# ReaganCardoza/Physics-Based-Ray-Tracing

Measured on AMD Instinct MI355X. Metric: Msamples/s on cbox.xml 512x512 x 256 spp (radiance, path max_depth 6), higher is better.
Workload: dtype f32

## Files before the change

include/pbrt_hip.h:

```cpp
#ifndef PBRT_HIP_H
#define PBRT_HIP_H

#include <stdint.h>

#ifdef __cplusplus
extern "C" {
#endif

#define PBRT_ABI_VERSION 5

#define PBRT_OK 0
#define PBRT_E_INVALID (-1)
#define PBRT_E_DEVICE (-2)
#define PBRT_E_NOMEM (-3)
#define PBRT_E_UNSUPPORTED (-4)

#define PBRT_PRIM_TRIANGLE 0u
#define PBRT_PRIM_SPHERE 1u
#define PBRT_PRIM_PARALLELOGRAM 2u
#define PBRT_PRIM_CONE 3u
#define PBRT_PRIM_CYLINDER 4u

typedef struct pbrt_prim {
    float g[12];
// ... 34 lines not shown
#define PBRT_ACCEL_BVH 2u
#define PBRT_ACCEL_BVH_GLOBAL 3u

typedef struct pbrt_scene_desc {
    uint32_t n_prims;
    const pbrt_prim *prims;
    uint32_t n_materials;
    const pbrt_material *materials;
    uint32_t n_emitters;
    const pbrt_emitter *emitters;
    uint32_t n_light_prims;
    const uint32_t *light_prims;
    const float *light_cdf;
    uint32_t accel;
    const float *vertex_normals;
} pbrt_scene_desc;

typedef struct pbrt_camera {
    float to_world[12];
    float tan_half_fov_x;
    float near_clip;
    float far_clip;
    uint32_t film_w;
    uint32_t film_h;
} pbrt_camera;

#define PBRT_FILTER_BOX 0u
#define PBRT_FILTER_TENT 1u
#define PBRT_FILTER_GAUSSIAN 2u

typedef struct pbrt_film_desc {
    uint32_t crop_x, crop_y, crop_w, crop_h;
    uint32_t spp;
    uint32_t sample_offset;
    uint32_t max_depth;
    uint32_t rr_depth;
    uint32_t filter;
    uint32_t seed;
    uint32_t flags;
    uint32_t pass_paths;
} pbrt_film_desc;

#define PBRT_FILM_RAW_ACCUM 1u
#define PBRT_FILM_NO_REPACK 2u
#define PBRT_FILM_FUSE_PLAN_SET 0x80u
#define PBRT_FILM_FUSE_PLAN(mask) (PBRT_FILM_FUSE_PLAN_SET | (((mask) & 0xffu) << 8))
#define PBRT_FILM_WALK_SET 0x10000u
#define PBRT_FILM_WALK_FROM(d) (PBRT_FILM_WALK_SET | (((d) & 0xffu) << 17))
#define PBRT_FILM_REGEN 8u
#define PBRT_FILM_NO_HIT_POOL 0x10u
#define PBRT_FILM_NO_OCCLUDER_PRUNING 4u
#define PBRT_FILM_NO_TILE_CULL 0x20u
#define PBRT_FILM_NO_ORDERED_WALK 0x40u

#define PBRT_US_MAX_ANGLES 64

typedef struct pbrt_us_emitter {
    uint32_t number_of_elements;
    float pitch, element_width, element_height;
    float radius;
    float opening_angle;
    uint32_t number_of_rays_per_element;
    float speed_of_sound;
    float steering_angle_min, steering_angle_max;
} pbrt_us_emitter;

#define PBRT_US_PRIMARY_ELEMENT 0u
#define PBRT_US_PRIMARY_EMITTER 1u
#define PBRT_US_ARRAY_CONVEX 0x100u

typedef struct pbrt_us_params {
    uint32_t max_depth;
    float frequency;
    float sound_speed;
    float attenuation;
    float main_beam_angle;
    float cutoff_angle;
    float fs;
    uint32_t n_elements;
    float pitch;
    uint32_t n_angles;
    float angles_deg[PBRT_US_MAX_ANGLES];
    uint32_t time_samples;
    float sensor_to_world[12];
    float max_path_len;
    uint32_t quirks;
    uint32_t primary;
    pbrt_us_emitter emitter;
} pbrt_us_params;

#define PBRT_USQ_DIAG_SAMPLE 0x1u
#define PBRT_USQ_REF_REFLECT 0x2u
#define PBRT_USQ_UNIT_GGX_PDF 0x4u
#define PBRT_USQ_DOUBLE_LOCAL 0x8u
#define PBRT_USQ_MIXED_FRAMES 0x10u
#define PBRT_USQ_NEVER_ENTER 0x20u
#define PBRT_USQ_CLAMP_TIME 0x40u
#define PBRT_USQ_NO_TOF_ACCUM 0x80u
#define PBRT_USQ_NO_CARRIER 0x100u
#define PBRT_USQ_NO_FIRST_TABLES 0x200u
#define PBRT_USQ_NO_FUSED_BOUNCES 0x400u
#define PBRT_USQ_FROZEN_DRAWS 0x800u
#define PBRT_USQ_SIGNED_RR 0x1000u
#define PBRT_USQ_DRJIT_VARIANT (PBRT_USQ_CLAMP_TIME | PBRT_USQ_NO_TOF_ACCUM | PBRT_USQ_FROZEN_DRAWS | PBRT_USQ_SIGNED_RR)
#define PBRT_USQ_REFERENCE                                                                \
    (PBRT_USQ_DIAG_SAMPLE | PBRT_USQ_REF_REFLECT | PBRT_USQ_UNIT_GGX_PDF | PBRT_USQ_DOUBLE_LOCAL | \
// ... 266 lines not shown
```

physics-based-ray-tracing_amd/_capi.py:

```python
from __future__ import annotations

import contextlib
import ctypes as C
import os
import sys

import numpy as np

_HERE = os.path.dirname(os.path.abspath(__file__))
LIB_PATH = os.environ.get("PBRT_HIP_LIB") or os.path.join(_HERE, "csrc", "libpbrt_hip.so")

PBRT_ABI_VERSION = 5

PRIM_TRIANGLE, PRIM_SPHERE, PRIM_PARALLELOGRAM, PRIM_CONE, PRIM_CYLINDER = 0, 1, 2, 3, 4
MAT_DIFFUSE, MAT_CONDUCTOR, MAT_DIELECTRIC, MAT_ULTRA, MAT_NONE = 0, 1, 2, 3, 4
MAT_ROUGHCONDUCTOR, MAT_CONDUCTOR_FRESNEL = 5, 6
EMIT_AREA, EMIT_POINT = 0, 1
ACCEL_AUTO, ACCEL_BRUTE, ACCEL_BVH, ACCEL_BVH_GLOBAL = 0, 1, 2, 3
FILTER_BOX, FILTER_TENT, FILTER_GAUSSIAN = 0, 1, 2
FILM_RAW_ACCUM = 1
FILM_NO_REPACK = 2
FILM_NO_OCCLUDER_PRUNING = 4
FILM_NO_TILE_CULL = 0x20
FILM_NO_ORDERED_WALK = 0x40
FILM_NO_HIT_POOL = 0x10
FILM_REGEN = 8
FILM_FUSE_PLAN_SET = 0x80


FILM_WALK_SET = 0x10000


def film_walk_from(depth: int) -> int:
    return FILM_WALK_SET | ((int(depth) & 0xFF) << 17)


def film_fuse_plan(mask: int) -> int:
    return FILM_FUSE_PLAN_SET | ((int(mask) & 0xFF) << 8)

US_MAX_ANGLES = 64

USQ_DIAG_SAMPLE = 0x1
USQ_REF_REFLECT = 0x2
USQ_UNIT_GGX_PDF = 0x4
USQ_DOUBLE_LOCAL = 0x8
USQ_MIXED_FRAMES = 0x10
USQ_NEVER_ENTER = 0x20
USQ_CLAMP_TIME = 0x40
USQ_NO_TOF_ACCUM = 0x80
USQ_NO_CARRIER = 0x100
USQ_NO_FIRST_TABLES = 0x200
USQ_NO_FUSED_BOUNCES = 0x400
USQ_FROZEN_DRAWS = 0x800
USQ_SIGNED_RR = 0x1000
USQ_DRJIT_VARIANT = USQ_CLAMP_TIME | USQ_NO_TOF_ACCUM | USQ_FROZEN_DRAWS | USQ_SIGNED_RR
USQ_REFERENCE = (USQ_DIAG_SAMPLE | USQ_REF_REFLECT | USQ_UNIT_GGX_PDF | USQ_DOUBLE_LOCAL
                 | USQ_MIXED_FRAMES | USQ_NEVER_ENTER)

PRIM_DTYPE = np.dtype([("g", np.float32, 12), ("type", np.uint32), ("material", np.uint32),
                       ("emitter", np.int32), ("shape", np.uint32)])
MATERIAL_DTYPE = np.dtype([("type", np.uint32), ("p", np.float32, 7)])
EMITTER_DTYPE = np.dtype([("type", np.uint32), ("radiance", np.float32, 3), ("pos", np.float32, 3),
                          ("first", np.uint32), ("count", np.uint32), ("area", np.float32),
                          ("pad", np.float32, 2)])
assert PRIM_DTYPE.itemsize == 64 and MATERIAL_DTYPE.itemsize == 32 and EMITTER_DTYPE.itemsize == 48


class Material(C.Structure):
    _fields_ = [("type", C.c_uint32), ("p", C.c_float * 7)]


class SceneDesc(C.Structure):
    _fields_ = [("n_prims", C.c_uint32), ("prims", C.c_void_p),
                ("n_materials", C.c_uint32), ("materials", C.c_void_p),
                ("n_emitters", C.c_uint32), ("emitters", C.c_void_p),
                ("n_light_prims", C.c_uint32), ("light_prims", C.c_void_p), ("light_cdf", C.c_void_p),
                ("accel", C.c_uint32), ("vertex_normals", C.c_void_p)]
# ... 500 lines not shown
```

physics-based-ray-tracing_amd/csrc/kernels_radiance.h:

```cpp
#pragma once
#include "device_scene.h"
#include "render_request.h"
#include "tile_cull.h"

#ifndef SEG_BRUTE
#define SEG_BRUTE 512
#endif
#ifndef SEG_BVH
#define SEG_BVH 1024
#endif
#ifndef SEG_WAVES_PER_EU
#define SEG_WAVES_PER_EU 8
#endif
#ifndef REGION_SEGS_BVH
#define REGION_SEGS_BVH 4
#endif
#ifndef REGION_SEGS_BRUTE
#define REGION_SEGS_BRUTE 1
#endif
#ifndef REGION_SEGS_US
#define REGION_SEGS_US 8
#endif
__host__ __device__ constexpr uint32_t rad_region_segs(int accel);
#ifndef REGION_SEGS_US_EMIT
// ... 36 lines not shown
    DevScene sc;
    pbrt_camera cam;
    const float *in;
    float *out;
    float *Lhome;
    const uint32_t *seg_in;
    uint32_t *seg_out;
    unsigned long long *stats;
    uint32_t stat_stride;
    uint32_t cap;
    uint32_t state_cap;
    uint32_t n_paths;
    uint32_t depth, max_depth, rr_depth, seed;
    uint32_t nb;
    uint32_t repack_mask;
    uint32_t merge_at;
    uint32_t key_mode;
    uint32_t rx0, ry0, rw, npix_r, s_first, film_w, film_h;
    uint32_t tile_rows;
    FastDiv div_npix, div_rw;
    uint32_t index_offset, sample_index;
    uint32_t lds_bytes;
    const uint32_t *tile_keep;
};

#define STATE_TILE_BYTES (64u * N_STATE * 4u)
#define STATE_ROW_BYTES 256u
DEV uint32_t state_voff(uint32_t slot) { return (slot >> 6) * STATE_TILE_BYTES + (slot & 63u) * 4u; }
typedef __amdgpu_buffer_rsrc_t Rsrc;
DEV Rsrc make_rsrc(const void *p, uint32_t bytes) {
    return __builtin_amdgcn_make_buffer_rsrc(const_cast<void *>(p), 0, bytes, 0x00020000);
}
DEV float bld(Rsrc r, uint32_t voff, uint32_t soff) {
    return __builtin_bit_cast(float, __builtin_amdgcn_raw_buffer_load_b32(r, voff, soff, 0));
}
DEV void bst(Rsrc r, uint32_t voff, uint32_t soff, float v) {
    __builtin_amdgcn_raw_buffer_store_b32(__builtin_bit_cast(uint32_t, v), r, voff, soff, 0);
}

DEV uint32_t region_index(uint32_t xx, uint32_t yy, uint32_t rw, uint32_t tile_rows) {
    return yy < tile_rows ? (yy >> 3) * (8u * rw) + (xx << 3) + (yy & 7u) : yy * rw + xx;
}

DEV uint32_t xcd_swizzle(uint32_t b, uint32_t n) {
    if ((b | 7u) >= n) return b;
    uint32_t g = b >> 3, rot = 0;
    while (g) {
        rot += g;
        g >>= 3;
    }
    return (b & ~7u) | ((b + rot) & 7u);
}

template <bool TILED>
DEV void path_key(const RadArgs &a, uint32_t home, uint32_t *ka, uint32_t *kb, uint32_t *px, uint32_t *py) {
    if (a.key_mode == 0) {
        uint32_t sl = udiv_fast(home, a.div_npix), pr = home - sl * a.npix_r;
        uint32_t rx, ry;
        if (TILED) {
            const bool tiled = pr < a.tile_rows * a.rw;
            const uint32_t num = tiled ? pr >> 3 : pr;
            const uint32_t q = udiv_fast(num, a.div_rw);
            rx = num - q * a.rw;
            ry = tiled ? (q << 3) + (pr & 7u) : q;
        } else {
            ry = udiv_fast(pr, a.div_rw);
            rx = pr - ry * a.rw;
        }
        *px = a.rx0 + rx;
        *py = a.ry0 + ry;
        *ka = *py * a.film_w + *px;
        *kb = a.s_first + sl;
    } else {
        *ka = a.index_offset + home;
        *kb = a.sample_index;
        *px = *py = 0;
    }
}

struct LdsScene {
    TreeLds tree;
    BvhStack stk;
};
#define NO_TREE_LDS TreeLds{nullptr, 0u, 0u}
#ifndef BVH_STK_ROWS
#define BVH_STK_ROWS 4
#endif
#define BVH_STK_DW(threads) (BVH_STK_ROWS * (threads))
__host__ __device__ constexpr uint32_t ilog2_c(uint32_t v) { return v <= 1u ? 0u : 1u + ilog2_c(v >> 1); }
#define MAKE_BVH_STACK(lds, threads) BvhStack{(LDS_AS uint32_t *)(lds) + threadIdx.x, ilog2_c(threads) + 0u, BVH_STK_ROWS}
#define BVH_STACK_LDS(ACCEL, THREADS)                                                                              \
    static_assert(((THREADS) & ((THREADS)-1)) == 0, "BVH stack rows are addressed by a shift");                    \
    __shared__ uint32_t bvh_stk_lds[((ACCEL) == ACCEL_K_BVH_GLOBAL || (ACCEL) == ACCEL_K_BVH_LDS) ? BVH_STK_DW(THREADS) : 1]
#define NO_LDS_SCENE {NO_TREE_LDS, BvhStack{nullptr, 0u, 0u}}

template <int ACCEL, bool ANY, bool SEGMENT = false, bool ORDERED = false>
DEV bool scene_intersect(const DevScene &sc, const LdsScene &ls, V3 o, V3 d, float tmax, Hit *h, uint32_t keep = 0xffffffffu) {
    static_assert(!ORDERED || ACCEL == ACCEL_K_BRUTE || ACCEL == ACCEL_K_BRUTE_BIG, "ordered walk: brute-force kernels only");
    if (ACCEL == ACCEL_K_BRUTE || ACCEL == ACCEL_K_BRUTE_BIG)
        return brute_intersect<ANY, SEGMENT, ACCEL != ACCEL_K_BRUTE, ORDERED>(sc, o, d, tmax, h, keep);
    if (ACCEL == ACCEL_K_BVH_GLOBAL) return bvh_intersect<ANY>(TreeGlobal{sc.nodes, sc.lprims}, sc.prims, ls.stk, o, d, tmax, h);
    return bvh_intersect<ANY>(ls.tree, sc.prims, ls.stk, o, d, tmax, h);
}

DEV void fill_tables_lds(const DevScene &sc, uint32_t *lds, uint32_t n_threads) {
    uint32_t *p_prims = lds, *p_mats = lds + TAB_MAX * 16, *p_emit = p_mats + TAB_MAX * 8, *p_lp = p_emit + TAB_MAX * 12;
    float *p_lc = reinterpret_cast<float *>(p_lp + TAB_MAX);
    for (uint32_t t = threadIdx.x; t < TAB_MAX * 16; t += n_threads) {
// ... 70 lines not shown
    }
    if (depth + 1 < a.max_depth) {
        const pbrt_material M = tb.mats[mat_id];
        Frame fr = make_frame(si.ns);
        V3 wi = to_local(fr, -d);
#ifdef PBRT_ABLATE_NEE
        if (false) {
#else
        if ((M.type == PBRT_MAT_DIFFUSE || (GLOSSY && M.type == PBRT_MAT_ROUGHCONDUCTOR)) && nE > 0) {
#endif
            F4 u = rng4(ka, kb, 1 + 2 * depth, a.seed);
            ESample es = sample_emitter(tb, si.p, u);
            if (es.valid) {
                V3 wo = to_local(fr, es.d);
                V3 f;
                float bpdf;
                bsdf_eval_pdf<GLOSSY>(M, wi, wo, &f, &bpdf);
                if (bpdf > 0.0f) {
                    V3 so = offset_origin(si.p, si.n, es.d);
                    V3 sv = es.q - so;
                    float sd = sqrtf(dot(sv, sv));
                    V3 sdir = sv * rcp_rn(sd);
                    if (segment(so, sdir, sd * (1.0f - K_SHADOW_EPS))) {
                        float mis = es.delta ? 1.0f : mis_weight(es.pdf, bpdf);
                        contribute(v3(thr.x * f.x, thr.y * f.y, thr.z * f.z), v3(es.weight.x * mis, es.weight.y * mis, es.weight.z * mis));
                    }
                }
            }
        }
        F4 ub = rng4(ka, kb, 2 + 2 * depth, a.seed);
        BSample bs = bsdf_sample<GLOSSY>(M, PBRT_USQ_REFERENCE, wi, si.n, si.ns, fr, ub.x, ub.y, ub.z);
        if (bs.valid) {
            thr = thr * bs.weight;
            eta *= bs.eta;
            V3 nd = to_world(fr, bs.wo);
            if (M.type == PBRT_MAT_ULTRA) nd = normalize(nd);
            o = offset_origin(si.p, si.n, nd);
            d = nd;
            prev_pdf = bs.delta ? -1.0f : bs.pdf;
            float tm = max3(thr);
            survive = true;
            if (depth + 1 >= a.rr_depth) {
                float q = fminf(tm * eta * eta, 0.95f);
                float rq = 1.0f / q;
                thr = thr * rq;
                if (!(ub.w < q)) survive = false;
            }
            if (tm == 0.0f) survive = false;
        }
    }
    return survive;
}

template <int ACCEL, bool HAVE_HIT = false, bool GLOSSY = ACCEL != ACCEL_K_BRUTE, bool ORDERED = false>
DEV bool bounce_step(const RadArgs &a, const Tables &tb, const LdsScene &ls, Rsrc r_L, uint32_t depth, uint32_t ka, uint32_t kb,
                     uint32_t home, float tmax, V3 &o, V3 &d, V3 &thr, V3 &L, float &eta, float &prev_pdf, bool &did_seg,
                     bool &did_shadow, const Hit *h_in = nullptr, uint32_t keep = 0xffffffffu) {
    bool survive = false;
    Hit h;
    if (HAVE_HIT) h = *h_in;
    if (HAVE_HIT || scene_intersect<ACCEL, false, false, ORDERED>(a.sc, ls, o, d, tmax, &h, keep)) {
        did_seg = true;
        const pbrt_prim &P = tb.prims_by_slot[h.slot];
        const SI si = make_si<ACCEL != ACCEL_K_BRUTE>(P, o, d, h.t, h.u, h.v, a.sc.vnormals, h.slot);
        survive = shade_step<GLOSSY>(
            a, tb, depth, ka, kb, h.t, P, si, o, d, thr, L, eta, prev_pdf,
            [&](V3 so, V3 sdir, float smax) {
                did_shadow = true;
#ifdef PBRT_ABLATE_SHADOW
                return smax > 0.0f;
#else
                Hit hs;
                return !scene_intersect<ACCEL, true, true, ORDERED>(a.sc, ls, so, sdir, smax, &hs);
#endif
            },
            [&](V3 A, V3 B) { L = {fma_(A.x, B.x, L.x), fma_(A.y, B.y, L.y), fma_(A.z, B.z, L.z)}; });
    }
    if (!survive) {
        typedef uint32_t __attribute__((ext_vector_type(4))) u32x4;
        const u32x4 rec = {__float_as_uint(L.x), __float_as_uint(L.y), __float_as_uint(L.z), 0u};
        __builtin_amdgcn_raw_buffer_store_b128(rec, r_L, home * 16u, 0, 0);
    }
    return survive;
}

template <bool FIRST, int ACCEL_T, int NB = 1>
#ifndef FUSED_WAVES_PER_EU
#define FUSED_WAVES_PER_EU 8
#endif
#ifndef GLOSSY_WAVES_PER_EU
#define GLOSSY_WAVES_PER_EU 4
#endif
__global__ __launch_bounds__(seg_threads(accel_base(ACCEL_T)), ACCEL_T == ACCEL_K_BRUTE_GLOSSY ? GLOSSY_WAVES_PER_EU : NB > 1 ? (accel_base(ACCEL_T) == ACCEL_K_BRUTE ? FUSED_WAVES_PER_EU : BIG_WAVES_PER_EU) : seg_waves_per_eu(accel_base(ACCEL_T))) void k_bounce(const RadArgs a) {
    constexpr int ACCEL = accel_base(ACCEL_T);
    static_assert(NB == 1 || ACCEL == ACCEL_K_BRUTE || ACCEL == ACCEL_K_BRUTE_BIG, "fused bounces: brute-force kernels only");
    constexpr bool GL = ACCEL_T == ACCEL_K_BRUTE_GLOSSY || ACCEL == ACCEL_K_BVH_GLOBAL || ACCEL == ACCEL_K_BVH_LDS;
    constexpr bool ORD = ACCEL_T == ACCEL_K_BRUTE_ORDERED;
    static_assert(NB == 1 || (rad_region_segs(ACCEL) == 1 && !rad_wave_private(ACCEL) && seg_threads(ACCEL) <= 1023),
                  "chain launches: REGION == SEG, workgroup scan");
    constexpr uint32_t SEG = seg_threads(ACCEL);
    extern __shared__ __attribute__((aligned(16))) uint32_t dyn_lds[];
    __shared__ uint32_t wave_tot[2][SEG / 64];
    __shared__ uint32_t wave_seg[2][SEG / 64];
    __shared__ uint32_t wave_shd[2][SEG / 64];
    __shared__ uint32_t wave_mid[2][NB > 1 ? SEG / 64 : 1], wave_mid_hi[2][NB > 1 ? SEG / 64 : 1];

    const uint32_t seg = xcd_swizzle(blockIdx.x, gridDim.x);
    const uint32_t tid = threadIdx.x;
    constexpr uint32_t REGION = rad_region_segs(ACCEL) * SEG;
    constexpr bool TILED = true;
    constexpr bool DYN = rad_dynamic(ACCEL);
    constexpr uint32_t W = SEG / 64;
    constexpr uint32_t CH = DYN ? 64u : SEG;
    const uint32_t lane_c = DYN ? (tid & 63u) : tid;
    const uint32_t row_id = DYN ? seg * W + (tid >> 6) : seg;
    const uint32_t base = seg * REGION;
    __shared__ uint32_t q_in, q_out, q_done;
    if (DYN && tid == 0) {
        q_in = 0;
        q_out = 0;
        q_done = 0;
    }
    uint32_t cnt_in;
    if (FIRST) {
        cnt_in = a.n_paths > base ? min(a.n_paths - base, REGION) : 0u;
    } else {
        cnt_in = a.seg_in[seg];
    }
    if (cnt_in == 0) {
        if (tid == 0) a.seg_out[seg] = 0;
        return;
// ... 158 lines not shown
        bst(r_out, v4 + 1 * row, 0, o.y);
        bst(r_out, v4 + 2 * row, 0, o.z);
        bst(r_out, v4 + 3 * row, 0, d.x);
        bst(r_out, v4 + 4 * row, 0, d.y);
        bst(r_out, v4 + 5 * row, 0, d.z);
        bst(r_out, v4 + 6 * row, 0, thr.x);
        bst(r_out, v4 + 7 * row, 0, thr.y);
        bst(r_out, v4 + 8 * row, 0, thr.z);
        bst(r_out, v4 + 9 * row, 0, L.x);
        bst(r_out, v4 + 10 * row, 0, L.y);
        bst(r_out, v4 + 11 * row, 0, L.z);
        bst(r_out, v4 + 12 * row, 0, eta);
        bst(r_out, v4 + 13 * row, 0, prev_pdf);
        bst(r_out, v4 + 14 * row, 0, __uint_as_float(home));
    }
    out_off += total;
    if (!DYN && tid == 0) {
        for (uint32_t w = 0; w < SEG / 64; ++w) {
            ns_acc += wave_seg[buf][w];
            nh_acc += wave_shd[buf][w];
            if (NB > 1) {
                mid_acc += wave_mid[buf][w];
                mid_acc_hi += wave_mid_hi[buf][w];
            }
        }
    }
    }
    if (DYN) {
        if ((tid & 63u) == 0) {
            unsigned long long *row = a.stats + row_id;
            const size_t stride = a.stat_stride;
            row[0] += ns_acc;
            row[stride] += nh_acc;
            row[(2 + min(a.depth, (uint32_t)MAX_DEPTH_STATS - 1)) * stride] += live_acc;
            if (atomicAdd(&q_done, 1u) == W - 1) a.seg_out[seg] = atomicAdd(&q_out, 0u);
        }
        return;
    }
    if (tid == 0) {
        a.seg_out[seg] = out_off;
        unsigned long long *row = a.stats + row_id;
        const size_t stride = a.stat_stride;
        row[0] += ns_acc;
        row[stride] += nh_acc;
        row[(2 + min(a.depth, (uint32_t)MAX_DEPTH_STATS - 1)) * stride] += cnt_in;
        if (NB > 1)
            for (uint32_t k = 1; k < nb_run; ++k) {
                const uint32_t n_on = k <= 3 ? (mid_acc >> (10u * (k - 1u))) & 1023u : (mid_acc_hi >> (10u * (k - 4u))) & 1023u;
                row[(2 + min(a.depth + k, (uint32_t)MAX_DEPTH_STATS - 1)) * stride] += n_on;
            }
    }
}

struct TileKeepArgs {
    const pbrt_prim *prims;
    uint32_t n_prims;
    pbrt_camera cam;
    uint32_t rx0, ry0, rw, tile_rows, n_blocks;
    FastDiv div_rw;
    uint32_t *keep;
};
__global__ __launch_bounds__(64) void k_tile_keep(const TileKeepArgs a) {
    const uint32_t blk = blockIdx.x * 64u + threadIdx.x;
    if (blk >= a.n_blocks) return;
    uint32_t x0 = 0xffffffffu, y0 = 0xffffffffu, x1 = 0, y1 = 0;
    for (uint32_t k = 0; k < 64u; ++k) {
        const uint32_t pr = blk * 64u + k;
        const bool tiled = pr < a.tile_rows * a.rw;
        const uint32_t num = tiled ? pr >> 3 : pr;
        const uint32_t q = udiv_fast(num, a.div_rw);
        const uint32_t rx = num - q * a.rw, ry = tiled ? (q << 3) + (pr & 7u) : q;
        x0 = min(x0, rx);
        x1 = max(x1, rx);
        y0 = min(y0, ry);
        y1 = max(y1, ry);
    }
    uint32_t word = 0;
    for (uint32_t i = 0; i < a.n_prims && i < 32u; ++i) {
        const pbrt_prim P = load_prim_uniform(a.prims + i);
        if (tile_cull_keep(a.cam, a.rx0 + x0, a.ry0 + y0, a.rx0 + x1, a.ry0 + y1, P)) word |= 1u << i;
    }
    word |= a.n_prims < 32u ? ~0u << a.n_prims : 0u;
    a.keep[blk] = word;
}

#define REDUCE_SLICES 32
__global__ __launch_bounds__(256) void k_reduce_stats(const unsigned long long *stats, uint32_t nseg, size_t stride,
                                                      unsigned long long *out) {
    __shared__ unsigned long long part[256];
    const unsigned long long *row = stats + (size_t)blockIdx.x * stride;
    const uint32_t per = (nseg + gridDim.y - 1) / gridDim.y, lo = min(blockIdx.y * per, nseg), hi = min(lo + per, nseg);
    unsigned long long s = 0;
    for (uint32_t i = lo + threadIdx.x; i < hi; i += 256) s += row[i];
    part[threadIdx.x] = s;
    __syncthreads();
    for (uint32_t w = 128; w > 0; w >>= 1) {
        if (threadIdx.x < w) part[threadIdx.x] += part[threadIdx.x + w];
        __syncthreads();
    }
    if (threadIdx.x == 0 && part[0]) atomicAdd(&out[blockIdx.x], part[0]);
}

__global__ __launch_bounds__(256) void k_us_reduce_stats(unsigned long long *stats, uint32_t nseg, size_t stride,
                                                         unsigned long long *out) {
    __shared__ unsigned long long part[4];
    unsigned long long *row = stats + (size_t)blockIdx.x * stride;
// ... 211 lines not shown
```

physics-based-ray-tracing_amd/csrc/pbrt_api.hip:

```cpp
#include <hip/hip_runtime.h>

#include <atomic>
#include <cmath>
#include <cstdarg>
#include <cstdio>
#include <cstring>
#include <map>
#include <numeric>
#include <string>
#include <tuple>
#include <vector>

#include "scene_request.h"
#include "bf_request.h"
#include "us_request.h"
#include "kernels_us.h"
#include "kernels_wavefront.h"
#include "kernels_us_wavefront.h"
#include "kernels_beamform.h"
#ifdef PBRT_DIAG
#include "kernels_diag.h"
#endif
#include "stage_layout.h"
#include "workspace.h"
// ... 109 lines not shown
    uint64_t serial = 0;
};

#define HIPCHK(ctx, call)                                                                              \
    do {                                                                                               \
        hipError_t e_ = (call);                                                                        \
        if (e_ != hipSuccess) return (ctx)->fail(PBRT_E_DEVICE, "%s: %s", #call, hipGetErrorString(e_)); \
    } while (0)
#define NEED(ctx, cond)                                                        \
    do {                                                                       \
        if (!(cond)) return (ctx)->fail(PBRT_E_INVALID, "invalid argument: %s", #cond); \
    } while (0)
#define MATERIAL_RULE(ctx, m, index)                                                                    \
    do {                                                                                                \
        Refusal why_;                                                                                   \
        if (int rc_ = material_rule(m, index, &why_)) return (ctx)->fail(rc_, "%s", why_.text);         \
    } while (0)

#define NOT_RECORDING(ctx)                                                                                                   \
    do {                                                                                                                     \
        if ((ctx)->recording) return (ctx)->refuse((std::string(__func__) + " cannot run").c_str());                         \
    } while (0)

static int us_finish(pbrt_ctx *c);
static inline int ctx_settle(pbrt_ctx *c) {
    if (c->recording) return c->refuse("only the queueing entry points may be called");
    return c->pend.active ? us_finish(c) : PBRT_OK;
}

template <typename T>
static int upload(pbrt_scene *s, const T *src, size_t n, const T **dst) {
    void *p = nullptr;
    size_t bytes = std::max<size_t>(n * sizeof(T), 16);
    HIPCHK(s->ctx, hipMalloc(&p, bytes));
    s->allocs.push_back(p);
    if (n) HIPCHK(s->ctx, hipMemcpy(p, src, n * sizeof(T), hipMemcpyHostToDevice));
    *dst = static_cast<const T *>(p);
    return PBRT_OK;
}


template <class F>
static auto with_flags(F f) { return f(); }
template <class F, class... Bs>
static auto with_flags(F f, bool b, Bs... rest) {
    auto bind = [&](auto c) { return with_flags([&](auto... cs) { return f(c, cs...); }, rest...); };
    return b ? bind(std::true_type{}) : bind(std::false_type{});
}
template <class K>
static hipError_t set_max_lds(K kernel, size_t bytes) {
    return hipFuncSetAttribute(reinterpret_cast<const void *>(kernel), hipFuncAttributeMaxDynamicSharedMemorySize, (int)bytes);
}
using RadKern = void (*)(RadArgs);
using WfKern = void (*)(WfArgs);
using UsKern = void (*)(UsArgs);
using UsWfKern = void (*)(UsWfArgs);
using UsFirstKern = void (*)(UsArgs, uint32_t, float4 *, float4 *);
using RayIntersectKern = void (*)(DevScene, uint32_t, const float *, const float *, const float *, float *, uint32_t *, float *, float *);
using RayTestKern = void (*)(DevScene, uint32_t, const float *, const float *, const float *, uint8_t *);

extern "C" {

int pbrt_abi_version(void) { return PBRT_ABI_VERSION; }

int pbrt_ctx_create(int device, pbrt_ctx **out) {
    if (!out) {
        g_ctxless_error = "pbrt_ctx_create: out is NULL";
        return PBRT_E_INVALID;
    }
    int n = 0;
    hipError_t e = hipGetDeviceCount(&n);
    if (e != hipSuccess || n == 0) {
        g_ctxless_error = std::string("no HIP device visible: ") + hipGetErrorString(e) +
                          " (the ray-transport hot path has no CPU fallback)";
        return PBRT_E_DEVICE;
    }
    if (device < 0 || device >= n) {
        g_ctxless_error = "device index out of range";
        return PBRT_E_INVALID;
    }
    pbrt_ctx *c = new pbrt_ctx();
    c->device = device;
#ifdef PBRT_CU_MASK_PROBE
    auto masked_stream = [&](hipStream_t *st) -> hipError_t {
        const char *m = getenv("PBRT_CU_MASK");
        if (!m) return hipStreamCreate(st);
        uint32_t mask[8] = {0, 0, 0, 0, 0, 0, 0, 0};
        for (uint32_t b = 0; b < 256; ++b) {
            bool on = !strcmp(m, "even") ? (b & 1u) == 0 : !strcmp(m, "odd") ? (b & 1u) == 1 : !strcmp(m, "low") ? b < 128
                      : !strcmp(m, "altcu") ? ((b >> 5) & 1u) == 0 : !strcmp(m, "altse") ? ((b >> 3) & 1u) == 0 : !strcmp(m, "altcu2") ? ((b >> 6) & 1u) == 0 : !strcmp(m, "pairs") ? (b & 2u) == 0 : true;
            if (on) mask[b >> 5] |= 1u << (b & 31u);
        }
        return hipExtStreamCreateWithCUMask(st, 8, mask);
    };
    if ((e = hipSetDevice(device)) != hipSuccess || (e = masked_stream(&c->stream)) != hipSuccess ||
#else
    if ((e = hipSetDevice(device)) != hipSuccess || (e = hipStreamCreate(&c->stream)) != hipSuccess ||
#endif
        (e = hipEventCreate(&c->ev0)) != hipSuccess || (e = hipEventCreate(&c->ev1)) != hipSuccess) {
        g_ctxless_error = std::string("device init: ") + hipGetErrorString(e);
        delete c;
        return PBRT_E_DEVICE;
    }
    if ((e = hipHostMalloc(&c->pinned, PIN_BYTES, hipHostMallocDefault)) != hipSuccess) {
        g_ctxless_error = std::string("hipHostMalloc: ") + hipGetErrorString(e);
        (void)hipStreamDestroy(c->stream);
// ... 207 lines not shown
    delete s;
    return PBRT_OK;
}

}

struct Switches {
    bool wf_packet = true;
    uint32_t wf_split_s = 0, wf_split_parts = 1;
    bool us_generic_kernel = false, us_emit_fused = true, env_general = false;
    int us_emit_permute = 1;
};
static Switches read_switches() {
    static const Switches once = [] {
        Switches w;
        if (const char *e = getenv("PBRT_WF_PACKET")) w.wf_packet = atoi(e) != 0;
        unsigned s_ = 0, p_ = 2;
        const char *e = getenv("PBRT_WF_SPLIT");
        if (e && sscanf(e, "%u%*[,:]%u", &s_, &p_) >= 1 && s_ >= 1 && s_ <= 7) {
            w.wf_split_s = s_;
            w.wf_split_parts = std::max(2u, std::min(p_, 8u));
        }
        return w;
    }();
    Switches w = once;
    auto flag = [](const char *name, bool unset) {
        const char *e = getenv(name);
        return e ? atoi(e) != 0 : unset;
    };
    w.us_generic_kernel = flag("PBRT_US_GENERIC_KERNEL", false);
    w.us_emit_fused = flag("PBRT_US_EMIT_FUSED", true);
    w.env_general = flag("PBRT_ENV_GENERAL", false);
    if (const char *e = getenv("PBRT_US_EMIT_PERMUTE")) w.us_emit_permute = atoi(e);
    return w;
}

static RadKern bounce_kernel(const pbrt_scene *s, bool first, uint32_t nb, bool ordered) {
    const bool two = nb >= 2;
    switch (s->accel_kernel) {
        case ACCEL_K_BRUTE:
            return with_flags([](auto F, auto O, auto N) -> RadKern {
                return &k_bounce<F(), O() ? ACCEL_K_BRUTE_ORDERED : ACCEL_K_BRUTE, N() ? 2 : 1>; }, first, ordered, two);
        case ACCEL_K_BRUTE_BIG:
            return with_flags([](auto F, auto G, auto N) -> RadKern {
                return &k_bounce<F(), G() ? ACCEL_K_BRUTE_GLOSSY : ACCEL_K_BRUTE_BIG, N() ? 2 : 1>; }, first, s->glossy, two);
        default:
            return nullptr;
    }
}
static int launch_bounce(pbrt_scene *s, const RadArgs &a, uint32_t nseg, bool first, uint32_t nb = 1) {
    const RadKern k = bounce_kernel(s, first, nb, a.sc.prim_ord != 0u);
    if (!k) return s->ctx->fail(PBRT_E_UNSUPPORTED, "launch_bounce: no fused bounce kernel for accelerator %d in this build", s->accel_kernel);
    hipLaunchKernelGGL(k, dim3(nseg), dim3(seg_threads(s->accel_kernel)), 0u, s->ctx->stream, a);
    return PBRT_OK;
}

static UsKern us_bounce_kernel(const pbrt_scene *s, bool first, bool emit, uint32_t q, int tab, bool convex = false) {
    if (!first) tab = -1;
    if (convex) {
        q = US_Q_RUNTIME;
        tab = -1;
    }
    switch (s->accel_kernel) {
        case ACCEL_K_BRUTE:
            if (q != US_Q_RUNTIME && (tab >= 0 || !first))
                return with_flags([](auto F, auto E, auto C, auto T) -> UsKern {
                    return &k_us_bounce<F(), ACCEL_K_BRUTE, E(), C() ? PBRT_USQ_REFERENCE : (PBRT_USQ_REFERENCE | PBRT_USQ_NO_CARRIER),
                                        !F() ? -1 : (!E() && T()) ? 1 : 0>; }, first, emit, q == PBRT_USQ_REFERENCE, tab == 1);
            return with_flags([](auto F, auto E, auto X) -> UsKern {
                return &k_us_bounce<F(), ACCEL_K_BRUTE, E(), US_Q_RUNTIME, -1, X()>; }, first, emit, convex);
        case ACCEL_K_BRUTE_BIG:
            return with_flags([](auto F, auto E, auto X) -> UsKern {
                return &k_us_bounce<F(), ACCEL_K_BRUTE_BIG, E(), US_Q_RUNTIME, -1, X()>; }, first, emit, convex);
        default:
            return nullptr;
    }
}


struct WfPlan {
    bool packet = true;
    uint32_t grid_deep = 2;
    uint32_t threads = 1024, rows = 2, grid_mult = 8;
    size_t lds = 0;
    uint32_t split_s = 0, split_parts = 1;
};
static WfPlan wf_plan(const pbrt_scene *s, const Switches &sw) {
    WfPlan p;
    const WfShape w = wf_shape(s->ctx->lds_limit, s->accel_kernel == ACCEL_K_BVH_LDS ? s->lds_bytes : 0u, s->bvh_depth, sw.wf_packet);
    p.threads = w.threads;
    p.rows = w.rows;
    p.lds = w.lds;
    p.packet = w.packet;
    p.split_s = sw.wf_split_s;
    p.split_parts = sw.wf_split_parts;
    return p;
}
struct TraceLaunch {
    WfKern kernel;
    uint32_t threads;
    size_t lds;
};
static TraceLaunch trace_kernel(const pbrt_scene *s, const WfPlan &p, bool first) {
    const bool lds = s->accel_kernel == ACCEL_K_BVH_LDS;
    if (first && p.packet) {
        auto primary = [](auto L, auto C) -> WfKern { return &k_trace_primary<L() ? ACCEL_K_BVH_LDS : ACCEL_K_BVH_GLOBAL, C()>; };
// ... 355 lines not shown
        hipLaunchKernelGGL((k_film_accum_tiled<8, PBRT_FILTER_TENT>), g8, dim3(8, 8), 0, st, fa);
    else
        hipLaunchKernelGGL((k_film_accum_tiled<8, PBRT_FILTER_GAUSSIAN>), g8, dim3(8, 8), 0, st, fa);
}

static int probe_plan(pbrt_ctx *c, unsigned long long *segstats, uint32_t n_rows, uint32_t stat_rows, unsigned long long *dstats,
                      uint32_t max_depth, uint32_t *plan) {
    hipStream_t st = c->stream;
    unsigned long long hp[2 + MAX_DEPTH_STATS];
    hipLaunchKernelGGL(k_reduce_stats, dim3(stat_rows, REDUCE_SLICES), dim3(256), 0, st, segstats, n_rows, (size_t)n_rows, dstats);
    HIPCHK(c, hipGetLastError());
    HIPCHK(c, hipMemcpyAsync(hp, dstats, (size_t)stat_rows * 8, hipMemcpyDeviceToHost, st));
    HIPCHK(c, hipStreamSynchronize(st));
    HIPCHK(c, hipMemsetAsync(dstats, 0, (2 + 2 * MAX_DEPTH_STATS) * 8, st));
    for (uint32_t d = stat_rows; d < 2 + MAX_DEPTH_STATS; ++d) hp[d] = 0;
    *plan = plan_from_survival(hp + 2, std::min<uint32_t>(max_depth, MAX_DEPTH_STATS));
    return PBRT_OK;
}

namespace {
struct Render {
    pbrt_scene *s;
    pbrt_ctx *c;
    const pbrt_camera *cam;
    const pbrt_film_desc *f;
    void *d_out;
    RenderRequest rq;
    Switches sw;
    PassShape ps;
    uint32_t n_own = 0, n_rows = 0;
    WfBufs wfb{};
    WfPlan wfp;
    float *Lhome = nullptr, *acc = nullptr;
    uint32_t *segA = nullptr, *segB = nullptr;
    unsigned long long *dstats = nullptr, *segstats = nullptr;
    FusePlan fp;
    RadArgs base{};
    FilmArgs fa{};
    PassTimer timer{};
    uint32_t passes = 0, launches = 0;
    unsigned long long hstats[2 + 2 * MAX_DEPTH_STATS];
    uint32_t hguard[WF_GUARD_WORDS] = {0};
};
}

static RenderLaunch render_launch(const pbrt_scene *s) {
    static_assert(WF_REGION == REGION_SEGS_BVH * SEG_BVH, "both BVH launch structures cut a pass into the same regions");
    const int k = s->accel_kernel;
    RenderLaunch l;
    l.brute = k == ACCEL_K_BRUTE || k == ACCEL_K_BRUTE_BIG;
    l.keep = k == ACCEL_K_BRUTE && s->ds.n_prims <= 32;
    l.region = rad_region_segs(k) * seg_threads(k);
    l.owners = rad_owners_per_region(k);
    l.rows_fused = rad_rows_per_region(k);
    l.rows_streams = WF_SHADE_THREADS / 64u;
    return l;
}

static int render_check(Render &r) {
    pbrt_ctx *c = r.c;
    if (int rcs = ctx_settle(c)) return rcs;
    if (const char *why = render_request(&r.rq, r.cam, r.f, r.d_out != nullptr, render_launch(r.s))) return RULE_TEXT(c, why);
    HIPCHK(c, hipSetDevice(c->device));
    r.sw = read_switches();
    return PBRT_OK;
}

static int render_buffers(Render &r) {
    pbrt_scene *s = r.s;
    pbrt_ctx *c = r.c;
    const pbrt_film_desc *f = r.f;
    const RenderRequest &rq = r.rq;
    const bool wavefront = rq.wavefront;
    const uint64_t pass_paths = f->pass_paths ? f->pass_paths
                                              : default_pass_paths(c, wavefront, rq.brute ? (64u << 20) : (16u << 20), 16 + 2 * N_STATE * 4);
    auto alloc_pass = [&](const PassShape &ps) -> int {
        r.Lhome = (float *)c->buf("Lhome", (size_t)ps.cap * 16);
        return r.Lhome && (!wavefront || wf_alloc(c, ps.cap, ps.nseg, &r.wfb)) ? PBRT_OK : PBRT_E_NOMEM;
    };
    int rc = size_pass(c, pass_paths, f->pass_paths != 0, f->spp, rq.npix_r, rq.launch.region, true, wavefront, N_STATE, alloc_pass, &r.ps);
    if (rc) return rc;
    if (wavefront) {
        r.wfp = wf_plan(s, r.sw);
        if ((rc = wf_set_attr(s, r.wfp)) != 0) return rc;
    }
    r.n_own = r.ps.nseg * rq.launch.owners;
    r.n_rows = r.ps.nseg * rq.rows_per_region();
    r.segA = (uint32_t *)c->buf("segA", (size_t)r.n_own * 4);
    r.segB = (uint32_t *)c->buf("segB", (size_t)r.n_own * 4);
    r.acc = (float *)c->buf("film_acc", rq.film_px * 16);
    r.dstats = (unsigned long long *)c->buf("stats", (2 + 2 * MAX_DEPTH_STATS) * 8);
    r.segstats = (unsigned long long *)c->buf("segstats", (size_t)(2 + 2 * MAX_DEPTH_STATS) * r.n_rows * 8);
    if (!r.segstats) return PBRT_E_NOMEM;
    return r.Lhome && r.segA && r.segB && r.acc && r.dstats ? PBRT_OK : PBRT_E_NOMEM;
}

static int render_clear(Render &r) {
    pbrt_ctx *c = r.c;
    const RenderRequest &rq = r.rq;
    hipStream_t st = c->stream;
    HIPCHK(c, hipMemsetAsync(r.acc, 0, rq.film_px * 16, st));
    HIPCHK(c, hipMemsetAsync(r.dstats, 0, (2 + 2 * MAX_DEPTH_STATS) * 8, st));
    HIPCHK(c, hipMemsetAsync(r.segstats, 0, (size_t)rq.stat_rows * r.n_rows * 8, st));
    if (rq.hit_rows) HIPCHK(c, hipMemsetAsync(r.segstats + (size_t)HIT_ROW0 * r.n_rows, 0, (size_t)rq.hit_rows * r.n_rows * 8, st));
    HIPCHK(c, hipEventRecord(c->ev0, st));
    r.timer = PassTimer{c};
    return PBRT_OK;
// ... 29 lines not shown
    base.key_mode = 0;
    render_film_args(r.rq, &base);
    base.div_npix = make_fastdiv(base.npix_r);
    base.div_rw = make_fastdiv(rw);
    const std::initializer_list<uint32_t> probes = {0u, 1u, rw - 1, rw, rw + 1, base.npix_r - 1, base.npix_r, base.npix_r + 1, cap - 1, cap, 0xffffffffu};
    NEED(r.c, fastdiv_exact(base.div_npix, base.npix_r, probes) && fastdiv_exact(base.div_rw, rw, probes));
    base.lds_bytes = s->lds_bytes;
    base.tile_keep = nullptr;
    return PBRT_OK;
}
static void render_film(Render &r) {
    const pbrt_film_desc *f = r.f;
    FilmArgs &fa = r.fa;
    fa.Lhome = r.Lhome;
    fa.acc = r.acc;
    fa.cap = r.ps.cap;
    fa.cx0 = f->crop_x;
    fa.cy0 = f->crop_y;
    fa.cw = f->crop_w;
    fa.ch = f->crop_h;
    render_film_args(r.rq, &fa);
    fa.rh = r.rq.rh;
    fa.filter = f->filter;
    fa.seed = f->seed;
}

static int render_tile_keep(Render &r) {
    pbrt_ctx *c = r.c;
    c->tile_keep_last = false;
    if (!r.rq.tile_keep) return PBRT_OK;
    TileKeepArgs ta;
    ta.prims = r.s->ds.prims;
    ta.n_prims = r.s->ds.n_prims;
    ta.cam = *r.cam;
    render_region_args(r.rq, &ta);
    ta.n_blocks = r.base.npix_r / 64;
    ta.div_rw = r.base.div_rw;
    ta.keep = (uint32_t *)c->buf("tile_keep", (size_t)ta.n_blocks * 4);
    if (!ta.keep) return PBRT_E_NOMEM;
    const pbrt_ctx::TileKeepKey key{c->work.generation("tile_keep"), r.s->serial, *r.cam, r.rq.rx0, r.rq.ry0, r.rq.rw, r.rq.rh};
    if (!(key == c->tile_keep_key)) {
        hipLaunchKernelGGL(k_tile_keep, dim3(div_up(ta.n_blocks, 64)), dim3(64), 0, c->stream, ta);
        HIPCHK(c, hipGetLastError());
        ++c->tile_keep_builds;
        c->tile_keep_key = key;
    }
    r.base.tile_keep = ta.keep;
    c->tile_keep_last = true;
    c->tile_keep_words = ta.keep;
    return PBRT_OK;
}

static int brute_bounces(pbrt_scene *s, RadArgs a, uint32_t plan, uint32_t nseg_pass, bool camera, uint32_t bound, float *in, float *out,
                         uint32_t *sin, uint32_t *sout, uint32_t n_own, uint32_t *launches) {
    pbrt_ctx *c = s->ctx;
    int rc;
    for (uint32_t depth = 0; depth < a.max_depth && depth < bound;) {
        const uint32_t nb = chain_len(plan, depth, a.max_depth);
        a.depth = depth;
        a.nb = nb;
        a.in = in;
        a.out = out;
        a.seg_in = sin;
        a.seg_out = sout;
        if ((rc = launch_bounce(s, a, nseg_pass, camera && depth == 0, nb)) != 0) return rc;
        HIPCHK(c, hipGetLastError());
        ++*launches;
        std::swap(in, out);
        std::swap(sin, sout);
        const uint32_t depth_before = depth;
        depth += nb;
        bool dead;
        if ((rc = poll_live(c, a.max_depth, depth_before, depth, sin, n_own, &dead)) != 0) return rc;
        if (dead) break;
    }
    return PBRT_OK;
}

constexpr uint32_t PASS_MAX_BOUNCES = 256;
static int brute_pass(Render &r, RadArgs a, uint32_t nseg_pass) {
    pbrt_ctx *c = r.c;
    const uint32_t region = r.rq.launch.region;
    const bool one_launch = chain_len(r.fp.plan, 0, a.max_depth) >= a.max_depth;
    const size_t need = one_launch ? (size_t)region : (size_t)nseg_pass * region;
    float *in = (float *)c->buf("stateA", need * N_STATE * 4), *out = (float *)c->buf("stateB", need * N_STATE * 4);
    if (!in || !out) return PBRT_E_NOMEM;
    a.state_cap = (uint32_t)need;
    if (int rc = r.timer.begin()) return rc;
    return brute_bounces(r.s, a, r.fp.plan, nseg_pass, true, PASS_MAX_BOUNCES, in, out, r.segA, r.segB, r.n_own, &r.launches);
}

static int render_passes(Render &r) {
    pbrt_ctx *c = r.c;
    const pbrt_film_desc *f = r.f;
    int rc;
    for (PassSchedule p{f->spp, r.ps.per_pass, r.fp.probe}; p.next(); ++r.passes) {
        RadArgs a = r.base;
        a.n_paths = (uint32_t)(r.rq.npix_r * p.sc);
        a.s_first = f->sample_offset + p.s0;
        const uint32_t nseg_pass = div_up(a.n_paths, r.rq.launch.region);
        if (r.rq.wavefront) {
            if ((rc = r.timer.begin()) != 0) return rc;
            rc = wf_bounces(r.s, wf_args(a), r.wfb, r.wfp, nseg_pass, true, &r.launches);
        } else {
            rc = brute_pass(r, a, nseg_pass);
        }
        if (rc) return rc;
        if ((rc = r.timer.end()) != 0) return rc;
        r.fa.s_first = a.s_first;
        r.fa.s_count = p.sc;
        film_accum(c, r.fa);
        HIPCHK(c, hipGetLastError());
        if (p.probing() && (rc = probe_plan(c, r.segstats, r.n_rows, r.rq.stat_rows, r.dstats, f->max_depth, &r.fp.plan)) != 0) return rc;
    }
    return PBRT_OK;
}

static int render_finish(Render &r) {
    pbrt_ctx *c = r.c;
    const RenderRequest &rq = r.rq;
    const uint32_t n_rows = r.n_rows;
    hipStream_t st = c->stream;
    int rc;
    hipLaunchKernelGGL(k_film_resolve, dim3(div_up(rq.film_px, 256)), dim3(256), 0, st, r.acc, (float *)r.d_out, (uint32_t)rq.film_px,
                       (uint32_t)(rq.out_floats == 4 ? 1 : 0));
    HIPCHK(c, hipGetLastError());
    HIPCHK(c, hipEventRecord(c->ev1, st));
    hipLaunchKernelGGL(k_reduce_stats, dim3(rq.stat_rows, REDUCE_SLICES), dim3(256), 0, st, r.segstats, n_rows, (size_t)n_rows, r.dstats);
    if (rq.hit_rows)
        hipLaunchKernelGGL(k_reduce_stats, dim3(rq.hit_rows, REDUCE_SLICES), dim3(256), 0, st, r.segstats + (size_t)HIT_ROW0 * n_rows, n_rows,
                           (size_t)n_rows, r.dstats + HIT_ROW0);
    HIPCHK(c, hipGetLastError());
    HIPCHK(c, hipMemcpyAsync(r.hstats, r.dstats, sizeof r.hstats, hipMemcpyDeviceToHost, st));
    if (rq.wavefront && (rc = wf_guard_fetch(c, r.hguard)) != 0) return rc;
    HIPCHK(c, hipStreamSynchronize(st));
    return rq.wavefront ? wf_check_guard(c, r.hguard) : PBRT_OK;
}

static int render_stats(Render &r) {
    pbrt_ctx *c = r.c;
    const unsigned long long *hstats = r.hstats;
    if (int rc = call_stats(c, hstats, r.rq.npix_r * r.f->spp, r.launches, r.passes, true, r.timer.n_ev)) return rc;
// ... 1343 lines not shown
```

Baseline: 11420.

## Add single-launch whole-path kernel for brute-force non-glossy scenes

New measurement: 11790, median of 6. 3.3% higher.

```diff
diff --git a/include/pbrt_hip.h b/include/pbrt_hip.h
--- a/include/pbrt_hip.h
+++ b/include/pbrt_hip.h
@@ -110,6 +110,7 @@
 #define PBRT_FILM_NO_OCCLUDER_PRUNING 4u
 #define PBRT_FILM_NO_TILE_CULL 0x20u
 #define PBRT_FILM_NO_ORDERED_WALK 0x40u
+#define PBRT_FILM_NO_PATH_KERNEL 0x2000000u
 
 #define PBRT_US_MAX_ANGLES 64
 
diff --git a/physics-based-ray-tracing_amd/_capi.py b/physics-based-ray-tracing_amd/_capi.py
--- a/physics-based-ray-tracing_amd/_capi.py
+++ b/physics-based-ray-tracing_amd/_capi.py
@@ -23,6 +23,7 @@
 FILM_NO_OCCLUDER_PRUNING = 4
 FILM_NO_TILE_CULL = 0x20
 FILM_NO_ORDERED_WALK = 0x40
+FILM_NO_PATH_KERNEL = 0x2000000
 FILM_NO_HIT_POOL = 0x10
 FILM_REGEN = 8
 FILM_FUSE_PLAN_SET = 0x80
diff --git a/physics-based-ray-tracing_amd/csrc/kernels_radiance.h b/physics-based-ray-tracing_amd/csrc/kernels_radiance.h
--- a/physics-based-ray-tracing_amd/csrc/kernels_radiance.h
+++ b/physics-based-ray-tracing_amd/csrc/kernels_radiance.h
@@ -112,8 +112,8 @@
     return (b & ~7u) | ((b + rot) & 7u);
 }
 
-template <bool TILED>
-DEV void path_key(const RadArgs &a, uint32_t home, uint32_t *ka, uint32_t *kb, uint32_t *px, uint32_t *py) {
+template <bool TILED, class Args>
+DEV void path_key(const Args &a, uint32_t home, uint32_t *ka, uint32_t *kb, uint32_t *px, uint32_t *py) {
     if (a.key_mode == 0) {
         uint32_t sl = udiv_fast(home, a.div_npix), pr = home - sl * a.npix_r;
         uint32_t rx, ry;
@@ -290,8 +290,8 @@
     return survive;
 }
 
-template <int ACCEL, bool HAVE_HIT = false, bool GLOSSY = ACCEL != ACCEL_K_BRUTE, bool ORDERED = false>
-DEV bool bounce_step(const RadArgs &a, const Tables &tb, const LdsScene &ls, Rsrc r_L, uint32_t depth, uint32_t ka, uint32_t kb,
+template <int ACCEL, bool HAVE_HIT = false, bool GLOSSY = ACCEL != ACCEL_K_BRUTE, bool ORDERED = false, bool STORE = true, class Args>
+DEV bool bounce_step(const Args &a, const Tables &tb, const LdsScene &ls, Rsrc r_L, uint32_t depth, uint32_t ka, uint32_t kb,
                      uint32_t home, float tmax, V3 &o, V3 &d, V3 &thr, V3 &L, float &eta, float &prev_pdf, bool &did_seg,
                      bool &did_shadow, const Hit *h_in = nullptr, uint32_t keep = 0xffffffffu) {
     bool survive = false;
@@ -314,7 +314,7 @@
             },
             [&](V3 A, V3 B) { L = {fma_(A.x, B.x, L.x), fma_(A.y, B.y, L.y), fma_(A.z, B.z, L.z)}; });
     }
-    if (!survive) {
+    if (STORE && !survive) {
         typedef uint32_t __attribute__((ext_vector_type(4))) u32x4;
         const u32x4 rec = {__float_as_uint(L.x), __float_as_uint(L.y), __float_as_uint(L.z), 0u};
         __builtin_amdgcn_raw_buffer_store_b128(rec, r_L, home * 16u, 0, 0);
@@ -579,6 +579,135 @@
     }
 }
 
+#ifndef PATH_THREADS
+#define PATH_THREADS 512
+#endif
+static_assert(SEG_BRUTE % PATH_THREADS == 0 && PATH_THREADS % 64 == 0, "a region of the brute-force kernels is whole k_path workgroups");
+__host__ __device__ constexpr uint32_t path_groups_per_region() { return SEG_BRUTE / PATH_THREADS; }
+struct PathArgs {
+    DevScene sc;
+    pbrt_camera cam;
+    float *Lhome;
+    unsigned long long *stats;
+    const uint32_t *tile_keep;
+    uint32_t stat_stride, cap, n_paths, max_depth, rr_depth, seed;
+    uint32_t rx0, ry0, rw, npix_r, s_first, film_w, film_h, tile_rows;
+    FastDiv div_npix, div_rw;
+    static constexpr uint32_t key_mode = 0, index_offset = 0, sample_index = 0;
+};
+static inline PathArgs path_args(const RadArgs &a) {
+    PathArgs p;
+    p.sc = a.sc;
+    p.cam = a.cam;
+    p.Lhome = a.Lhome;
+    p.stats = a.stats;
+    p.tile_keep = a.tile_keep;
+    p.stat_stride = a.stat_stride;
+    p.cap = a.cap;
+    p.n_paths = a.n_paths;
+    p.max_depth = a.max_depth;
+    p.rr_depth = a.rr_depth;
+    p.seed = a.seed;
+    p.rx0 = a.rx0;
+    p.ry0 = a.ry0;
+    p.rw = a.rw;
+    p.npix_r = a.npix_r;
+    p.s_first = a.s_first;
+    p.film_w = a.film_w;
+    p.film_h = a.film_h;
+    p.tile_rows = a.tile_rows;
+    p.div_npix = a.div_npix;
+    p.div_rw = a.div_rw;
+    return p;
+}
+template <int ACCEL_T, int THREADS>
+__global__ __launch_bounds__(THREADS, FUSED_WAVES_PER_EU) void k_path(const PathArgs a) {
+    static_assert(ACCEL_T == ACCEL_K_BRUTE || ACCEL_T == ACCEL_K_BRUTE_ORDERED, "k_path: ACCEL_K_BRUTE scenes without glossy materials");
+    constexpr bool ORD = ACCEL_T == ACCEL_K_BRUTE_ORDERED;
+    constexpr uint32_t W = THREADS / 64;
+    __shared__ uint32_t tab_lds[TAB_DW];
+    __shared__ uint32_t wg_cnt[2 + MAX_CHAIN];
+    const uint32_t wg = xcd_swizzle(blockIdx.x, gridDim.x);
+    const uint32_t tid = threadIdx.x;
+    const uint32_t base = wg * THREADS;
+    if (base >= a.n_paths) return;
+    const uint32_t cnt_in = min(a.n_paths - base, (uint32_t)THREADS);
+    if (tid < 2 + MAX_CHAIN) wg_cnt[tid] = 0;
+    const LdsScene ls = NO_LDS_SCENE;
+    const Tables tb = stage_tables_lds(a.sc, tab_lds);
+    fill_tables_lds(a.sc, tab_lds, THREADS);
+
+    const bool alive = tid < cnt_in;
+    const uint32_t home = base + tid;
+    V3 o = {0, 0, 0}, d = {0, 0, 1}, thr = {1, 1, 1}, L = {0, 0, 0};
+    float eta = 1.0f, prev_pdf = -1.0f, tmax = K_INF;
+    uint32_t ka = 0, kb = 0, px = 0, py = 0;
+    if (alive) {
+        path_key<true>(a, home, &ka, &kb, &px, &py);
+        F4 uj = rng4(ka, kb, 0, a.seed);
+        float fx = (float)px + uj.x, fy = (float)py + uj.y;
+        camera_ray(a.cam, film_coord(fx, a.film_w), film_coord(fy, a.film_h), &o, &d, &tmax);
+    }
+    uint32_t keep = 0xffffffffu;
+    if (a.tile_keep) {
+        const uint32_t home0 = base + ((uint32_t)__builtin_amdgcn_readfirstlane((int)tid) & ~63u);
+        const uint32_t blk = (home0 - udiv_fast(home0, a.div_npix) * a.npix_r) >> 6;
+        keep = load_uniform<uint32_t>(a.tile_keep + min(blk, (a.npix_r >> 6) - 1u));
+    }
+    bool live = alive;
+    uint32_t nseg_w = 0, nshd_w = 0;
+    unsigned long long non_w = 0;
+    static_assert(8 * (MAX_CHAIN - 1) <= 64, "the per-bounce counts of a wave (<= 64 each) are packed 8 bits each");
+    const uint32_t nb_run = min(a.max_depth, (uint32_t)MAX_CHAIN);
+#pragma unroll 1
+    for (uint32_t depth = 0; depth < nb_run; ++depth) {
+        if (depth > 0) {
+            const uint32_t n_on = (uint32_t)__popcll(__ballot(live));
+            if (n_on == 0) break;
+            non_w += (unsigned long long)n_on << (8u * (depth - 1u));
+            tmax = K_INF;
+        }
+        bool did_seg = false, did_shadow = false, survive = false;
+        if (live)
+            survive = bounce_step<ACCEL_K_BRUTE, false, false, ORD, false>(a, tb, ls, Rsrc(), depth, ka, kb, home, tmax, o, d, thr, L, eta, prev_pdf,
+                                                                           did_seg, did_shadow, nullptr, keep);
+        keep = 0xffffffffu;
+        live = survive;
+        nseg_w += (uint32_t)__popcll(__ballot(did_seg));
+        nshd_w += (uint32_t)__popcll(__ballot(did_shadow));
+    }
+    if (alive) {
+        typedef uint32_t __attribute__((ext_vector_type(4))) u32x4;
+        const u32x4 rec = {__float_as_uint(L.x), __float_as_uint(L.y), __float_as_uint(L.z), 0u};
+        __builtin_amdgcn_raw_buffer_store_b128(rec, make_rsrc(a.Lhome, a.cap * 16u), home * 16u, 0, 0);
+    }
+    if ((tid & 63u) == 0) {
+        if (nseg_w) atomicAdd(&wg_cnt[0], nseg_w);
+        if (nshd_w) atomicAdd(&wg_cnt[1], nshd_w);
+#pragma unroll
+        for (uint32_t k = 1; k < MAX_CHAIN; ++k) {
+            const uint32_t n_on = (uint32_t)(non_w >> (8u * (k - 1u))) & 255u;
+            if (n_on) atomicAdd(&wg_cnt[1 + k], n_on);
+        }
+        __builtin_amdgcn_fence(__ATOMIC_RELEASE, "workgroup");
+        if (atomicAdd(&wg_cnt[1 + MAX_CHAIN], 1u) == W - 1) {
+            __builtin_amdgcn_fence(__ATOMIC_ACQUIRE, "workgroup");
+            unsigned long long *row = a.stats + wg;
+            const size_t stride = a.stat_stride;
+            unsigned long long v[2 + MAX_CHAIN];
+            uint32_t add[2 + MAX_CHAIN];
+#pragma unroll
+            for (uint32_t k = 0; k < 2 + MAX_CHAIN; ++k) {
+                add[k] = k == 2 ? cnt_in : atomicAdd(&wg_cnt[k < 2 ? k : k - 1], 0u);
+                if (k < 2 + nb_run) v[k] = row[k * stride];
+            }
+#pragma unroll
+            for (uint32_t k = 0; k < 2 + MAX_CHAIN; ++k)
+                if (k < 2 + nb_run) row[k * stride] = v[k] + add[k];
+        }
+    }
+}
+
 struct TileKeepArgs {
     const pbrt_prim *prims;
     uint32_t n_prims;
diff --git a/physics-based-ray-tracing_amd/csrc/pbrt_api.hip b/physics-based-ray-tracing_amd/csrc/pbrt_api.hip
--- a/physics-based-ray-tracing_amd/csrc/pbrt_api.hip
+++ b/physics-based-ray-tracing_amd/csrc/pbrt_api.hip
@@ -185,6 +185,7 @@
     return hipFuncSetAttribute(reinterpret_cast<const void *>(kernel), hipFuncAttributeMaxDynamicSharedMemorySize, (int)bytes);
 }
 using RadKern = void (*)(RadArgs);
+using PathKern = void (*)(PathArgs);
 using WfKern = void (*)(WfArgs);
 using UsKern = void (*)(UsArgs);
 using UsWfKern = void (*)(UsWfArgs);
@@ -498,6 +499,18 @@
     const RadKern k = bounce_kernel(s, first, nb, a.sc.prim_ord != 0u);
     if (!k) return s->ctx->fail(PBRT_E_UNSUPPORTED, "launch_bounce: no fused bounce kernel for accelerator %d in this build", s->accel_kernel);
     hipLaunchKernelGGL(k, dim3(nseg), dim3(seg_threads(s->accel_kernel)), 0u, s->ctx->stream, a);
+    return PBRT_OK;
+}
+static PathKern path_kernel(const pbrt_scene *s, bool ordered) {
+    if (s->accel_kernel != ACCEL_K_BRUTE || s->glossy) return nullptr;
+    return with_flags([](auto O) -> PathKern { return &k_path<O() ? ACCEL_K_BRUTE_ORDERED : ACCEL_K_BRUTE, PATH_THREADS>; }, ordered);
+}
+static int launch_path(pbrt_scene *s, PathKern k, const RadArgs &a, uint32_t nseg) {
+    pbrt_ctx *c = s->ctx;
+    const uint32_t groups = nseg * path_groups_per_region();
+    NEED(c, a.key_mode == 0 && a.depth == 0 && a.max_depth <= MAX_CHAIN && a.stat_stride >= groups && (uint64_t)groups * PATH_THREADS <= a.cap);
+    HIPCHK(c, hipMemsetAsync(a.seg_out, 0, (size_t)nseg * 4, c->stream));
+    hipLaunchKernelGGL(k, dim3(groups), dim3(PATH_THREADS), 0u, c->stream, path_args(a));
     return PBRT_OK;
 }
 
@@ -959,7 +972,7 @@
     l.keep = k == ACCEL_K_BRUTE && s->ds.n_prims <= 32;
     l.region = rad_region_segs(k) * seg_threads(k);
     l.owners = rad_owners_per_region(k);
-    l.rows_fused = rad_rows_per_region(k);
+    l.rows_fused = k == ACCEL_K_BRUTE ? std::max(rad_rows_per_region(k), path_groups_per_region()) : rad_rows_per_region(k);
     l.rows_streams = WF_SHADE_THREADS / 64u;
     return l;
 }
@@ -1095,7 +1108,7 @@
 }
 
 static int brute_bounces(pbrt_scene *s, RadArgs a, uint32_t plan, uint32_t nseg_pass, bool camera, uint32_t bound, float *in, float *out,
-                         uint32_t *sin, uint32_t *sout, uint32_t n_own, uint32_t *launches) {
+                         uint32_t *sin, uint32_t *sout, uint32_t n_own, uint32_t *launches, bool path_ok = false) {
     pbrt_ctx *c = s->ctx;
     int rc;
     for (uint32_t depth = 0; depth < a.max_depth && depth < bound;) {
@@ -1106,7 +1119,8 @@
         a.out = out;
         a.seg_in = sin;
         a.seg_out = sout;
-        if ((rc = launch_bounce(s, a, nseg_pass, camera && depth == 0, nb)) != 0) return rc;
+        const PathKern whole = path_ok && camera && depth == 0 && nb >= a.max_depth ? path_kernel(s, a.sc.prim_ord != 0u) : nullptr;
+        if ((rc = whole ? launch_path(s, whole, a, nseg_pass) : launch_bounce(s, a, nseg_pass, camera && depth == 0, nb)) != 0) return rc;
         HIPCHK(c, hipGetLastError());
         ++*launches;
         std::swap(in, out);
@@ -1130,7 +1144,8 @@
     if (!in || !out) return PBRT_E_NOMEM;
     a.state_cap = (uint32_t)need;
     if (int rc = r.timer.begin()) return rc;
-    return brute_bounces(r.s, a, r.fp.plan, nseg_pass, true, PASS_MAX_BOUNCES, in, out, r.segA, r.segB, r.n_own, &r.launches);
+    return brute_bounces(r.s, a, r.fp.plan, nseg_pass, true, PASS_MAX_BOUNCES, in, out, r.segA, r.segB, r.n_own, &r.launches,
+                         !(r.f->flags & PBRT_FILM_NO_PATH_KERNEL));
 }
 
 static int render_passes(Render &r) {
```
